# SysSec-KAIST/LTESniffer

Hardware: AMD Instinct MI355X
Metric: subframes/s (20 MHz, 150 RNTIs) (higher is better)
Workload: dtype f32+int16

## Files before the change

ltesniffer_amd/csrc/kernels/lsn_dsp.h:

```cpp
#pragma once
#include "lsn_dev.h"

__device__ __forceinline__ cf32 cmul(cf32 a, cf32 b) { cf32 c; c.r = a.r * b.r - a.i * b.i; c.i = a.r * b.i + a.i * b.r; return c; }
__device__ __forceinline__ cf32 cmulconj(cf32 a, cf32 b) { cf32 c; c.r = a.r * b.r + a.i * b.i; c.i = a.i * b.r - a.r * b.i; return c; }
__device__ __forceinline__ float cabs2(cf32 a) { return a.r * a.r + a.i * a.i; }

template <int R>
__device__ __forceinline__ void fft_pass(cf32* a, const cf32* w, int s, int N, int lgN, int tid)
{
  constexpr int G = 1 << R;
  const int h = 1 << s;
#pragma unroll
  for (int u = 0; u < (8 >> R); u++) {
    int g = tid * (8 >> R) + u;
    if (g >= (N >> R)) break;
    int low = g & (h - 1), high = g >> s, base = (high << (s + R)) | low;
    cf32 e[G];
#pragma unroll
    for (int j = 0; j < G; j++) e[j] = a[base + j * h];
#pragma unroll
    for (int q = 0; q < R; q++) {
#pragma unroll
      for (int j = 0; j < G; j++) {
        if (j & (1 << q)) continue;
        int pos = low + (j & ((1 << q) - 1)) * h;
        cf32 v = cmul(e[j + (1 << q)], w[pos << (lgN - (s + q + 1))]);
        cf32 uu = e[j];
        e[j].r = uu.r + v.r; e[j].i = uu.i + v.i;
        e[j + (1 << q)].r = uu.r - v.r; e[j + (1 << q)].i = uu.i - v.i;
      }
    }
#pragma unroll
    for (int j = 0; j < G; j++) a[base + j * h] = e[j];
  }
}
template <int NB>
__device__ __forceinline__ void fft_passes(cf32* a, const cf32* w, int M, int lgN, int tid)
{
  for (int s = 0; s < lgN;) {
    const int left = lgN - s;
    if (left >= 3) { for (int r = 0; r < NB; r++) fft_pass<3>(a + r * M, w, s, M, lgN, tid); s += 3; }
    else if (left == 2) { for (int r = 0; r < NB; r++) fft_pass<2>(a + r * M, w, s, M, lgN, tid); s += 2; }
    else { for (int r = 0; r < NB; r++) fft_pass<1>(a + r * M, w, s, M, lgN, tid); s += 1; }
    __syncthreads();
  }
}
template <typename Load>
__device__ __forceinline__ void lsn_symbol_fft(const LsnCellDev& c, cf32* a, cf32* w, Load load, cf32* out, int dc, int tid)
{
  const int N = (int)c.N, lgN = (int)c.lgN, nre = (int)c.nre;
  if (c.twiddle3) {
    const int M = (int)c.nsub;
    for (int n = tid; n < M / 2; n += 256) w[n] = c.twiddle[n];
    for (int n = tid; n < N; n += 256) {
      const cf32 x = load(n);
      const int m = n / 3, r = n - 3 * m;
      a[r * M + (int)(__brev((unsigned)m) >> (32 - lgN))] = x;
    }
    __syncthreads();
    fft_passes<3>(a, w, M, lgN, tid);
    const cf32* __restrict__ T = c.twiddle3;
    for (int k = tid; k < nre; k += 256) {
      const int bin = (k < nre / 2) ? (N - nre / 2 + k) : (k - nre / 2 + dc), kq = bin & (M - 1);
      int b2 = 2 * bin;
      b2 = b2 >= N ? b2 - N : b2;
      const cf32 t1 = cmul(a[M + kq], T[bin]), t2 = cmul(a[2 * M + kq], T[b2]);
      const float sr = a[kq].r + t1.r, si = a[kq].i + t1.i;
      cf32 X;
      X.r = sr + t2.r;
      X.i = si + t2.i;
      out[k] = X;
    }
    return;
  }
  for (int n = tid; n < N / 2; n += 256) w[n] = c.twiddle[n];
  for (int n = tid; n < N; n += 256) a[__brev((unsigned)n) >> (32 - lgN)] = load(n);
  __syncthreads();
  fft_passes<1>(a, w, N, lgN, tid);
  for (int k = tid; k < nre; k += 256) out[k] = a[(k < nre / 2) ? (N - nre / 2 + k) : (k - nre / 2 + dc)];
}

__device__ __forceinline__ void lsn_demod_llr(int Qm, float I, float Q, float* L)
{
  float aI = fabsf(I), aQ = fabsf(Q);
  L[0] = -I; L[1] = -Q;
  if (Qm == 4) {
    const float a = 0.31622776601683794f;
    L[2] = aI - 2.0f * a; L[3] = aQ - 2.0f * a;
  } else if (Qm == 6) {
    const float a = 0.15430334996209191f;
    float tI = aI - 4.0f * a, tQ = aQ - 4.0f * a;
    L[2] = tI; L[3] = tQ; L[4] = fabsf(tI) - 2.0f * a; L[5] = fabsf(tQ) - 2.0f * a;
  } else if (Qm == 8) {
    const float a = 0.07669649888473704f;
    float tI = aI - 8.0f * a, tQ = aQ - 8.0f * a;
    float uI = fabsf(tI) - 4.0f * a, uQ = fabsf(tQ) - 4.0f * a;
    L[2] = tI; L[3] = tQ; L[4] = uI; L[5] = uQ; L[6] = fabsf(uI) - 2.0f * a; L[7] = fabsf(uQ) - 2.0f * a;
  }
}
```

ltesniffer_amd/csrc/kernels/stage_a.hip:

```cpp
#include "lsn_dsp.h"
#include <algorithm>
#include <type_traits>
#include <cstdlib>

#define SQRT2F 1.41421356237309504880f

__device__ __forceinline__ void ofdm_rb_power(const LsnCellDev& c, const cf32* out, float* __restrict__ rbp_part, int sf, int l, int tid)
{
  __syncthreads();
  if (tid < (int)c.nof_prb) {
    float s = 0.0f;
    for (int k = 0; k < 12; k++) { const cf32 x = out[tid * 12 + k]; s = s + (x.r * x.r + x.i * x.i); }
    rbp_part[((size_t)sf * 14 + l) * 128 + tid] = s / 12.0f;
  }
}
__global__ __launch_bounds__(256) void k_ofdm(LsnCellDev c, const cf32* __restrict__ iq, const uint32_t* __restrict__ dphi_sf,
                                              cf32* __restrict__ grid, float* __restrict__ rbp_part)
{
  extern __shared__ __attribute__((aligned(16))) unsigned char smem[];
  const int N = (int)c.N, tid = threadIdx.x;
  cf32* a = (cf32*)smem;
  cf32* w = a + N;
  const int nsym = (int)c.nsym;
  const int blk = blockIdx.x, l = blk % nsym, rx = (blk / nsym) % (int)c.nof_rx, sf = blk / (nsym * (int)c.nof_rx);
  const int cp0 = 160 * N / 2048, cp1 = 144 * N / 2048;
  const int slot = l / 7, ls = l % 7;
  const int pos = c.cp ? l * (N + N / 4) + N / 4 : slot * (cp0 + 6 * cp1 + 7 * N) + cp0 + ls * (N + cp1);
  const cf32* in = iq + ((size_t)sf * c.iq_nant + rx) * c.sflen + pos;
  const uint32_t dphi = dphi_sf ? dphi_sf[sf] : 0u;
  const int nre = (int)c.nre;
  cf32* out = grid + (((size_t)sf * c.nof_rx + rx) * 14 + l) * nre;
  auto load = [&](int n) {
    cf32 x = in[n];
    if (dphi != 0u) {
      uint32_t ph = (uint32_t)(pos + n) * dphi;
      cf32 rot = cmul(c.nco_coarse[ph >> 20], c.nco_fine[(ph >> 10) & 1023u]);
      x = cmul(x, rot);
    }
    return x;
  };
  lsn_symbol_fft(c, a, w, load, out, 1, tid);
  if (rbp_part && rx == 0) ofdm_rb_power(c, out, rbp_part, sf, l, tid);
}

void lsn_launch_ofdm(const LsnCellDev& c, const cf32* iq, const uint32_t* dphi, cf32* grid, uint32_t nsf, hipStream_t s, float* rbp_part)
{
  size_t lds = sizeof(cf32) * (c.N + c.N / 2);
  LSN_LAUNCH(k_ofdm, dim3(nsf * c.nof_rx * c.nsym), dim3(256), lds, s, c, iq, dphi, grid, rbp_part);
}

__device__ __forceinline__ int crs_koff(const LsnCellDev& c, int port, int s)
{
  int v = (port == 0) ? ((s & 1) ? 3 : 0) : (port == 1) ? ((s & 1) ? 0 : 3) : (port == 2) ? 3 * s : 3 + 3 * s;
  return (v + (int)(c.id % 6)) % 6;
}

__global__ __launch_bounds__(256) void k_chest(LsnCellDev c, const cf32* __restrict__ grid, const uint32_t* __restrict__ sf_idx_arr,
                                               cf32* __restrict__ ce, float* __restrict__ raw)
{
  extern __shared__ __attribute__((aligned(16))) unsigned char smem[];
  const int nre = (int)c.nre, nref = (int)c.nref, tid = threadIdx.x;
  const int P = (int)c.nof_ports, A = (int)c.nof_rx;
  const int blk = blockIdx.x, p = blk % P, rx = (blk / P) % A, sf = blk / (P * A);
  cf32* ls = (cf32*)smem;
  cf32* sm = ls + 4 * nref;
  float* part = (float*)(sm + 4 * nref);
  const int S = p < 2 ? 4 : 2;
  const int nsl = (int)c.nslot, nsym = (int)c.nsym;
  const int sym[4] = {p < 2 ? 0 : 1, p < 2 ? nsl - 3 : nsl + 1, nsl, 2 * nsl - 3};
  const cf32* g = grid + ((size_t)sf * A + rx) * 14 * nre;
  const cf32* crs = c.crs + ((size_t)sf_idx_arr[sf] * P + p) * 4 * nref;
  const int n4 = S * nref;
  for (int i = tid; i < n4; i += 256) {
    int s = i / nref, m = i - s * nref;
    ls[i] = cmulconj(g[sym[s] * nre + 6 * m + crs_koff(c, p, s)], crs[i]);
  }
  __syncthreads();
  for (int i = tid; i < n4; i += 256) {
    int s = i / nref, m = i - s * nref;
    float ar = 0.0f, ai = 0.0f;
#pragma unroll
    for (int j = 0; j < 5; j++) {
      int q = m + j - 2;
      if (q < 0 || q >= nref) continue;
      ar = ar + c.taps[j] * ls[s * nref + q].r;
      ai = ai + c.taps[j] * ls[s * nref + q].i;
    }
    sm[i].r = ar; sm[i].i = ai;
  }
  __syncthreads();
  float p0 = 0.0f, p1 = 0.0f, p2 = 0.0f, p3 = 0.0f, p4 = 0.0f, p5 = 0.0f;
  for (int i = tid; i < n4; i += 256) {
    float dr = sm[i].r - ls[i].r, di = sm[i].i - ls[i].i;
    p0 = p0 + (dr * dr + di * di);
    p1 = p1 + ls[i].r;
    p2 = p2 + ls[i].i;
    p3 = p3 + (sm[i].r * sm[i].r + sm[i].i * sm[i].i);
  }
  if (p < 2)
    for (int i = tid; i < 2 * nref; i += 256) {
      cf32 t = (i < nref) ? cmulconj(ls[2 * nref + i], ls[i]) : cmulconj(ls[3 * nref + (i - nref)], ls[nref + (i - nref)]);
      p4 = p4 + t.r;
      p5 = p5 + t.i;
    }
  part[0 * 256 + tid] = p0; part[1 * 256 + tid] = p1; part[2 * 256 + tid] = p2;
  part[3 * 256 + tid] = p3; part[4 * 256 + tid] = p4; part[5 * 256 + tid] = p5;
  __syncthreads();
  for (int s = 128; s > 0; s >>= 1) {
    if (tid < s) {
#pragma unroll
      for (int q = 0; q < 6; q++) part[q * 256 + tid] = part[q * 256 + tid] + part[q * 256 + tid + s];
    }
    __syncthreads();
  }
  if (tid < 6) raw[(((size_t)sf * A + rx) * P + p) * 8 + tid] = part[tid * 256];
  cf32* co = ce + (((size_t)sf * P + p) * A + rx) * 14 * nre;
  for (int k = tid; k < nre; k += 256) {
    cf32 row[4];
#pragma unroll
    for (int s = 0; s < 4; s++) {
      if (s >= S) break;
      int koff = crs_koff(c, p, s);
      const cf32* pl = sm + s * nref;
      int m = (k - koff) >= 0 ? (k - koff) / 6 : 0;
      if (m > nref - 2) m = nref - 2;
      float dr = (pl[m + 1].r - pl[m].r) / 6.0f, di = (pl[m + 1].i - pl[m].i) / 6.0f;
      float f = (float)(k - (6 * m + koff));
      row[s].r = pl[m].r + dr * f;
      row[s].i = pl[m].i + di * f;
    }
    if (p >= 2) {
      const cf32 c1 = row[0], c8 = row[1];
      const int la = sym[0], lb = sym[1];
      const float dl = (float)(lb - la);
      const float dr = (c8.r - c1.r) / dl, di = (c8.i - c1.i) / dl;
      co[la * nre + k] = c1; co[lb * nre + k] = c8;
      for (int l = 0; l < nsym; l++) {
        if (l == la || l == lb) continue;
        cf32 v; v.r = c1.r + dr * (float)(l - la); v.i = c1.i + di * (float)(l - la); co[l * nre + k] = v;
      }
      continue;
    }
    cf32 c0 = row[0], c4 = row[1], c7 = row[2], c11 = row[3];
    const int q0 = sym[0], q1 = sym[1], q2 = sym[2], q3 = sym[3];
    const float w01 = (float)(q1 - q0), w12 = (float)(q2 - q1), w23 = (float)(q3 - q2);
    float d01r = (c4.r - c0.r) / w01, d01i = (c4.i - c0.i) / w01;
    float d12r = (c7.r - c4.r) / w12, d12i = (c7.i - c4.i) / w12;
    float d23r = (c11.r - c7.r) / w23, d23i = (c11.i - c7.i) / w23;
    co[q0 * nre + k] = c0; co[q1 * nre + k] = c4; co[q2 * nre + k] = c7; co[q3 * nre + k] = c11;
    for (int l = q0 + 1; l < q1; l++) { cf32 v; v.r = c0.r + d01r * (float)(l - q0); v.i = c0.i + d01i * (float)(l - q0); co[l * nre + k] = v; }
    for (int l = q1 + 1; l < q2; l++) { cf32 v; v.r = c4.r + d12r * (float)(l - q1); v.i = c4.i + d12i * (float)(l - q1); co[l * nre + k] = v; }
    for (int l = q2 + 1; l < q3; l++) { cf32 v; v.r = c7.r + d23r * (float)(l - q2); v.i = c7.i + d23i * (float)(l - q2); co[l * nre + k] = v; }
    for (int l = q3 + 1; l < nsym; l++) { cf32 v; v.r = c11.r + d23r * (float)(l - q3); v.i = c11.i + d23i * (float)(l - q3); co[l * nre + k] = v; }
  }
}

void lsn_launch_chest(const LsnCellDev& c, const cf32* grid, const uint32_t* sf_idx, cf32* ce, float* raw, uint32_t nsf, hipStream_t s)
{
  size_t lds = sizeof(cf32) * 8 * c.nref + sizeof(float) * 6 * 256;
  LSN_LAUNCH(k_chest, dim3(nsf * c.nof_rx * c.nof_ports), dim3(256), lds, s, c, grid, sf_idx, ce, raw);
}

__global__ void k_chest_fin(LsnCellDev c, const float* __restrict__ raw, LsnChest* __restrict__ out, uint32_t nsf)
{
  uint32_t sf = blockIdx.x * blockDim.x + threadIdx.x;
  if (sf >= nsf) return;
  const int A = (int)c.nof_rx, P = (int)c.nof_ports;
  LsnChest o;
  float ns = 0.0f, rs = 0.0f, cp = 0.0f, cr = 0.0f, ci = 0.0f;
  for (int q = 0; q < LSN_MAX_RX * LSN_MAX_PORTS; q++) { o.noise[q] = 0.0f; o.rsrp[q] = 0.0f; o.cepow[q] = 0.0f; }
  for (int rx = 0; rx < A; rx++)
    for (int p = 0; p < P; p++) {
      const float* r = raw + (((size_t)sf * A + rx) * P + p) * 8;
      const float n = (float)((p < 2 ? 4 : 2) * c.nref);
      float noise = r[0] / n, mr = r[1] / n, mi = r[2] / n, cepow = r[3] / n;
      float rsrp = mr * mr + mi * mi;
      o.noise[rx * P + p] = noise; o.rsrp[rx * P + p] = rsrp; o.cepow[rx * P + p] = cepow;
      ns = ns + noise; rs = rs + rsrp; cp = cp + cepow;
      cr = cr + r[4]; ci = ci + r[5];
    }
  float cnt = (float)(A * P);
  o.noise_avg = ns / cnt; o.rsrp_avg = rs / cnt; o.chan_ref = cp; o.corr_r = cr; o.corr_i = ci;
  o.pad[0] = o.pad[1] = o.pad[2] = 0.0f;
  out[sf] = o;
}
void lsn_launch_chest_fin(const LsnCellDev& c, const float* raw, LsnChest* out, uint32_t nsf, hipStream_t s)
{
  LSN_LAUNCH(k_chest_fin, dim3((nsf + 63) / 64), dim3(64), 0, s, c, raw, out, nsf);
}

__device__ __forceinline__ void reg_equalise(const LsnCellDev& c, const cf32* __restrict__ g, const cf32* __restrict__ ce, float noise,
                                             int l, int k0, cf32* x, int rs, int ps)
{
  const int A = (int)c.nof_rx;
  int kk[4], n = 0;
  if ((c.reg_w6 >> l) & 1u) {
    for (int k = k0; k < k0 + 6; k++)
      if ((k % 3) != (int)(c.id % 3)) { if (n < 4) kk[n] = k; n++; }
  } else {
    for (int k = 0; k < 4; k++) kk[k] = k0 + k;
  }
  if (c.nof_ports == 1) {
#pragma unroll
    for (int i = 0; i < 4; i++) {
      float nr = 0.0f, ni = 0.0f, den = 0.0f;
      for (int rx = 0; rx < A; rx++) {
        cf32 y = g[rx * rs + kk[i]];
        cf32 h = ce[rx * rs + kk[i]];
        cf32 t = cmulconj(y, h);
        float hp = h.r * h.r + h.i * h.i;
        if (rx == 0) { nr = t.r; ni = t.i; den = hp; } else { nr = nr + t.r; ni = ni + t.i; den = den + hp; }
      }
      den = den + noise;
      x[i].r = nr / den; x[i].i = ni / den;
    }
  } else {
#pragma unroll
    for (int i = 0; i < 4; i += 2) {
      float x0r = 0, x0i = 0, x1r = 0, x1i = 0, hh = 0;
      const int pa = (c.nof_ports == 4 && i == 2) ? 1 : 0, pb = c.nof_ports == 4 ? pa + 2 : 1;
      for (int rx = 0; rx < A; rx++) {
        const int bg = rx * rs, b0 = pa * ps + rx * rs, b1 = pb * ps + rx * rs;
        cf32 r0 = g[bg + kk[i]], r1 = g[bg + kk[i + 1]];
        cf32 h00 = ce[b0 + kk[i]], h01 = ce[b0 + kk[i + 1]], h10 = ce[b1 + kk[i]], h11 = ce[b1 + kk[i + 1]];
        float hp = (h00.r * h00.r + h00.i * h00.i) + (h11.r * h11.r + h11.i * h11.i);
        cf32 a = cmulconj(r0, h00), b = cmulconj(h11, r1), cc = cmulconj(h10, r0), d = cmulconj(r1, h01);
        float t0r = a.r + b.r, t0i = a.i + b.i, t1r = d.r - cc.r, t1i = d.i - cc.i;
        if (rx == 0) { x0r = t0r; x0i = t0i; x1r = t1r; x1i = t1i; hh = hp; }
        else { x0r = x0r + t0r; x0i = x0i + t0i; x1r = x1r + t1r; x1i = x1i + t1i; hh = hh + hp; }
      }
      x[i].r = x0r / hh * SQRT2F; x[i].i = x0i / hh * SQRT2F;
      x[i + 1].r = x1r / hh * SQRT2F; x[i + 1].i = x1i / hh * SQRT2F;
    }
  }
}

__global__ __launch_bounds__(64) void k_pcfich(LsnCellDev c, const cf32* __restrict__ grid, const cf32* __restrict__ ce,
                                               const LsnChest* __restrict__ ch, const uint32_t* __restrict__ sf_idx_arr,
                                               uint32_t* __restrict__ cfi_out, float* __restrict__ corr_out)
{
  __shared__ float llr[32];
  const int sf = blockIdx.x, lane = threadIdx.x;
  const cf32* g = grid + (size_t)sf * c.nof_rx * 14 * c.nre;
  const cf32* e = ce + (size_t)sf * c.nof_ports * c.nof_rx * 14 * c.nre;
  const uint8_t* scr = c.pcfich_scr + sf_idx_arr[sf] * 32;
  if (lane < 4) {
    cf32 x[4];
    reg_equalise(c, g, e, ch[sf].noise_avg, 0, (int)c.pcfich_k0[lane], x, 14 * (int)c.nre, (int)c.nof_rx * 14 * (int)c.nre);
    for (int j = 0; j < 4; j++) {
      float a = -(x[j].r * SQRT2F), b = -(x[j].i * SQRT2F);
      llr[8 * lane + 2 * j] = scr[8 * lane + 2 * j] ? -a : a;
      llr[8 * lane + 2 * j + 1] = scr[8 * lane + 2 * j + 1] ? -b : b;
    }
  }
  __syncthreads();
  if (lane == 0) {
    uint32_t best = 0; float bestc = 0.0f;
    for (int w = 0; w < 3; w++) {
      float acc = 0.0f;
      for (int i = 0; i < 32; i++) acc = acc + (((i % 3) != w) ? llr[i] : -llr[i]);
      corr_out[sf * 3 + w] = acc;
      if (w == 0 || acc > bestc) { bestc = acc; best = (uint32_t)w; }
    }
    cfi_out[sf] = best + 1;
  }
}
void lsn_launch_pcfich(const LsnCellDev& c, const cf32* grid, const cf32* ce, const LsnChest* ch, const uint32_t* sf_idx, uint32_t* cfi, float* corr, uint32_t nsf, hipStream_t s)
{
  LSN_LAUNCH(k_pcfich, dim3(nsf), dim3(64), 0, s, c, grid, ce, ch, sf_idx, cfi, corr);
}

__global__ __launch_bounds__(256) void k_pdcch_llr(LsnCellDev c, const cf32* __restrict__ grid, const cf32* __restrict__ ce,
                                                   const LsnChest* __restrict__ ch, const uint32_t* __restrict__ sf_idx_arr,
                                                   const uint32_t* __restrict__ cfi_arr, float* __restrict__ llr)
{
  const int sf = blockIdx.y;
  const uint32_t cfi = cfi_arr[sf];
  const int nre = (int)c.nre, A = (int)c.nof_rx, n0 = nre / 6, n1 = nre / 4;
  const int nat = blockIdx.x * 256 + threadIdx.x;
  int l = 0, k0 = 0, r = nat;
  for (;; l++) {
    const int six = (int)((c.reg_w6 >> l) & 1u), cnt = six ? n0 : n1;
    if (r < cnt || l == 3) { k0 = (six ? 6 : 4) * r; break; }
    r -= cnt;
  }
  if (k0 >= nre) return;
  if ((uint32_t)l >= cfi + (c.nof_prb <= 10 ? 1u : 0u) || nat >= 800) return;
  const uint32_t q = c.reg_q[(cfi - 1) * 800 + nat];
  if (q >= c.nof_cce[cfi - 1] * 9) return;
  const cf32* g = grid + ((size_t)sf * A * 14 + l) * nre;
  const cf32* e = ce + ((size_t)sf * c.nof_ports * A * 14 + l) * nre;
  const uint8_t* sc = c.pdcch_scr + (size_t)sf_idx_arr[sf] * LSN_LLR_STRIDE + 8 * q;
  cf32 x[4];
  reg_equalise(c, g, e, ch[sf].noise_avg, l, k0, x, 14 * nre, A * 14 * nre);
  float v[8];
#pragma unroll
  for (int j = 0; j < 4; j++) {
    float a = -(x[j].r * SQRT2F), b = -(x[j].i * SQRT2F);
    v[2 * j] = sc[2 * j] ? -a : a;
    v[2 * j + 1] = sc[2 * j + 1] ? -b : b;
  }
  float4 o0, o1;
  o0.x = v[0]; o0.y = v[1]; o0.z = v[2]; o0.w = v[3]; o1.x = v[4]; o1.y = v[5]; o1.z = v[6]; o1.w = v[7];
  float4* o = reinterpret_cast<float4*>(llr + (size_t)sf * LSN_LLR_STRIDE + 8 * q);
  o[0] = o0; o[1] = o1;
}
void lsn_launch_pdcch_llr(const LsnCellDev& c, const cf32* grid, const cf32* ce, const LsnChest* ch, const uint32_t* sf_idx, const uint32_t* cfi, float* llr, uint32_t nsf, hipStream_t s)
{
  const uint32_t nreg = c.nre / 6 + (c.nof_prb <= 10 ? 3u : 2u) * (c.nre / 4);
  LSN_LAUNCH(k_pdcch_llr, dim3((nreg + 255) / 256, nsf), dim3(256), 0, s, c, grid, ce, ch, sf_idx, cfi, llr);
}

__global__ __launch_bounds__(128) void k_cce_power(LsnCellDev c, const float* __restrict__ llr, const uint32_t* __restrict__ cfi_arr,
                                                   float* __restrict__ pw)
{
  const int sf = blockIdx.x, cce = threadIdx.x;
  if (cce >= LSN_CCE_STRIDE) return;
  float out = 0.0f;
  if ((uint32_t)cce < c.nof_cce[cfi_arr[sf] - 1]) {
    const float* l = llr + (size_t)sf * LSN_LLR_STRIDE + 72 * cce;
    double mean = 0.0;
    for (int i = 0; i < 72; i++) mean += (double)fabsf(l[i]);
    out = (float)(mean / 72.0);
  }
  pw[sf * LSN_CCE_STRIDE + cce] = out;
}
void lsn_launch_cce_power(const LsnCellDev& c, const float* llr, const uint32_t* cfi, float* pw, uint32_t nsf, hipStream_t s)
{
  LSN_LAUNCH(k_cce_power, dim3(nsf), dim3(128), 0, s, c, llr, cfi, pw);
}

__device__ __forceinline__ uint32_t ss_validate(uint32_t n, uint32_t ncce, uint32_t l, uint32_t nsubframe, uint32_t rnti)
{
  const bool ue = rnti >= 0x000Bu && rnti <= 0xFFF3u;
  if (!ue && !((rnti >= 1u && rnti <= 10u) || rnti >= 0xFFFDu)) return 0;
  uint32_t Yk = rnti;
  if (ue)
    for (uint32_t m = 0; m <= nsubframe; m++) {
      const uint32_t x = 39827u * Yk;
      const int t = (int)(x & 0xFFFFu) - (int)(x >> 16);
      Yk = (uint32_t)(t < 0 ? t + 65537 : t);
    }
  auto member = [&](uint32_t lv) -> bool {
    const uint32_t L = 1u << lv;
    if (n < L) return false;
    if (lv >= 2) {
      const uint32_t lim = (n < 16u ? n : 16u) / L;
      if ((ncce & (L - 1)) == 0 && ncce / L < lim && ncce + L <= n) return true;
    }
    if (!ue || (ncce & (L - 1))) return false;
// ... 499 lines not shown
```

ltesniffer_amd/csrc/kernels/stage_ul.hip:

```cpp
#include "lsn_dsp.h"

#define LLR_Q 180.0f

__global__ __launch_bounds__(256) void k_ul_fft(LsnCellDev c, const cf32* __restrict__ iq, uint32_t nant, uint32_t ant, cf32* __restrict__ grid)
{
  extern __shared__ __attribute__((aligned(16))) unsigned char smem[];
  const int N = (int)c.N, tid = threadIdx.x;
  cf32* a = (cf32*)smem;
  cf32* w = a + N;
  const int nsym = (int)c.nsym;
  const int l = blockIdx.x % nsym, sf = blockIdx.x / nsym;
  const int cp0 = 160 * N / 2048, cp1 = 144 * N / 2048;
  const int slot = l / 7, ls = l % 7;
  const int pos = c.cp ? l * (N + N / 4) + N / 4 : slot * (cp0 + 6 * cp1 + 7 * N) + cp0 + ls * (N + cp1);
  const cf32* in = iq + ((size_t)sf * nant + ant) * c.sflen + pos;
  const int nre = (int)c.nre;
  cf32* out = grid + ((size_t)sf * 14 + l) * nre;
  lsn_symbol_fft(c, a, w, [&](int n) { return cmul(in[n], c.ul_shift[n]); }, out, 0, tid);
}

void lsn_launch_ul_fft(const LsnCellDev& c, const cf32* iq, uint32_t nant, uint32_t ant, cf32* grid, uint32_t nsf, hipStream_t s)
{
  LSN_LAUNCH(k_ul_fft, dim3(nsf * c.nsym), dim3(256), sizeof(cf32) * (c.N + c.N / 2), s, c, iq, nant, ant, grid);
}

__global__ __launch_bounds__(256) void k_pusch_chest(LsnCellDev c, const LsnUlGrantDev* __restrict__ grants, const cf32* __restrict__ grid,
                                                     cf32* __restrict__ hs_out, float* __restrict__ stat)
{
  extern __shared__ __attribute__((aligned(16))) unsigned char smem[];
  const LsnUlGrantDev g = grants[blockIdx.x];
  const int M = 12 * (int)g.L_prb, nre = (int)c.nre, tid = threadIdx.x;
  cf32* ls = (cf32*)smem;
  float* part = (float*)(ls + 2 * M);
  for (int i = tid; i < 2 * M; i += 256) {
    const int s = i >= M ? 1 : 0, n = i - s * M;
    const cf32 y = grid[((size_t)g.sf * 14 + (c.nslot - 4) + c.nslot * s) * nre + 12 * (s ? g.n_prb2 : g.n_prb) + n];
    const cf32 r = cmul(c.ul_base[(s ? g.base_off1 : g.base_off) + n], c.ul_ph12[(g.ncs[s] * (uint32_t)n) % 12u]);
    ls[i] = cmulconj(y, r);
  }
  __syncthreads();
  cf32* hs = hs_out + g.hs_off;
  float p0 = 0.0f, p1 = 0.0f;
  for (int i = tid; i < 2 * M; i += 256) {
    const int s = i >= M ? 1 : 0, n = i - s * M;
    const cf32* q = ls + s * M;
    cf32 a;
    if (n == 0) { a.r = (q[0].r + q[1].r) / 2.0f; a.i = (q[0].i + q[1].i) / 2.0f; }
    else if (n == M - 1) { a.r = (q[n - 1].r + q[n].r) / 2.0f; a.i = (q[n - 1].i + q[n].i) / 2.0f; }
    else { a.r = ((q[n - 1].r + q[n].r) + q[n + 1].r) / 3.0f; a.i = ((q[n - 1].i + q[n].i) + q[n + 1].i) / 3.0f; }
    hs[i] = a;
    const float dr = a.r - q[n].r, di = a.i - q[n].i;
    p0 = p0 + (dr * dr + di * di);
    p1 = p1 + (a.r * a.r + a.i * a.i);
  }
  part[tid] = p0; part[256 + tid] = p1;
  __syncthreads();
  for (int s = 128; s > 0; s >>= 1) {
    if (tid < s) { part[tid] = part[tid] + part[tid + s]; part[256 + tid] = part[256 + tid] + part[256 + tid + s]; }
    __syncthreads();
  }
  if (tid == 0) {
    stat[2 * blockIdx.x] = part[0] / (float)(2 * M);
    stat[2 * blockIdx.x + 1] = part[256] / (float)(2 * M);
  }
}

void lsn_launch_pusch_chest(const LsnCellDev& c, const LsnUlGrantDev* g, const cf32* grid, cf32* hs, float* stat, uint32_t ngrants, hipStream_t s)
{
  LSN_LAUNCH(k_pusch_chest, dim3(ngrants), dim3(256), sizeof(cf32) * 2 * 1200 + sizeof(float) * 512, s, c, g, grid, hs, stat);
}

__global__ __launch_bounds__(256) void k_pusch_demod(LsnCellDev c, const LsnUlGrantDev* __restrict__ grants, const cf32* __restrict__ grid,
                                                     const cf32* __restrict__ hs_all, const float* __restrict__ stat, int16_t* __restrict__ llr)
{
  extern __shared__ __attribute__((aligned(16))) unsigned char smem[];
  const LsnUlGrantDev g = grants[blockIdx.y];
  const int nsl = (int)c.nslot, dm = nsl - 4, ncol = 2 * (nsl - 1);
  const int col = blockIdx.x, l = col < dm ? col : (col < nsl - 1 + dm ? col + 1 : col + 2);
  const int M = 12 * (int)g.L_prb, nre = (int)c.nre, Qm = (int)g.qm, tid = threadIdx.x;
  cf32* xa = (cf32*)smem;
  cf32* xb = xa + M;
  cf32* w = xb + M;
  const cf32* y = grid + ((size_t)g.sf * 14 + l) * nre + 12 * (l >= nsl ? g.n_prb2 : g.n_prb);
  const cf32* h = hs_all + g.hs_off + (l >= nsl ? 1 : 0) * M;
  const cf32* wt = c.ul_idft + g.idft_off;
  const float noise = stat[2 * blockIdx.y];
  for (int n = tid; n < M; n += 256) {
    const cf32 hh = h[n], t = cmulconj(y[n], hh);
    const float den = (hh.r * hh.r + hh.i * hh.i) + noise;
    cf32 v; v.r = t.r / den; v.i = t.i / den;
    xa[n] = v;
    w[n] = wt[n];
  }
  __syncthreads();
  cf32 *in = xa, *out = xb;
  for (int n = M, s = 1; n > 1;) {
    const int r = (n % 4 == 0) ? 4 : (n % 2 == 0) ? 2 : (n % 3 == 0) ? 3 : 5;
    const int m = n / r, wr = M / r;
    for (int o = tid; o < M; o += 256) {
      const int q = o % s, rest = o / s, t = rest % r, p = rest / r;
      cf32 acc = cmul(in[q + s * p], w[0]);
      int wi = 0;
      for (int i = 1; i < r; i++) {
        wi += t * wr; wi = wi >= M ? wi - M : wi;
        const cf32 term = cmul(in[q + s * (p + m * i)], w[wi]);
        acc.r = acc.r + term.r; acc.i = acc.i + term.i;
      }
      out[o] = cmul(acc, w[(int)(((unsigned)p * (unsigned)t * (unsigned)s) % (unsigned)M)]);
    }
    __syncthreads();
    cf32* sw = in; in = out; out = sw;
    n = m; s *= r;
  }
  const float scale = g.scale;
  int16_t* e = llr + g.llr_off;
  for (int r = tid; r < M; r += 256) {
    const float ar = in[r].r, ai = in[r].i;
    int dcell; bool is_ack = false;
    {
      const int qri = (int)g.q_ri, qack = (int)g.q_ack, qcqi = (int)g.q_cqi;
      auto in_col = [&](int q, int slot) { const int i0 = (4 - slot) & 3; return q > i0 ? (q - 1 - i0) / 4 + 1 : 0; };
      int before = 0; bool is_ri = false;
#pragma unroll
      for (int slot = 0; slot < 4; slot++) {
        const int cc = c.cp ? (slot == 0 ? 0 : (slot == 1 ? 3 : (slot == 2 ? 5 : 8))) : (slot == 0 ? 1 : (slot == 1 ? 4 : (slot == 2 ? 7 : 10))), n = in_col(qri, slot), top = M - n;
        before += r > top ? r - top : 0;
        if (n && r >= top && cc < col) before += 1;
        if (n && r >= top && cc == col) is_ri = true;
        const int ca = c.cp ? (slot == 0 ? 1 : (slot == 1 ? 2 : (slot == 2 ? 6 : 7))) : (slot == 0 ? 2 : (slot == 1 ? 3 : (slot == 2 ? 8 : 9)));
        if (ca == col && r >= M - in_col(qack, slot) && in_col(qack, slot)) is_ack = true;
      }
      const int rank = r * ncol + col - before;
      dcell = (is_ri || rank < qcqi) ? -1 : rank - qcqi;
    }
    float Lb[8];
    lsn_demod_llr(Qm, ar * scale, ai * scale, Lb);
#pragma unroll
    for (int b = 0; b < 8; b++) {
      if (b >= Qm) break;
      float v = rintf(Lb[b] * LLR_Q);
      v = v > (float)LSN_LLR_CLIP ? (float)LSN_LLR_CLIP : v;
      v = v < (float)-LSN_LLR_CLIP ? (float)-LSN_LLR_CLIP : v;
      int q = (int)v;
      const uint32_t sidx = ((uint32_t)col * (uint32_t)M + (uint32_t)r) * (uint32_t)Qm + (uint32_t)b;
      const uint32_t cbit = (uint32_t)c.gold_x1[sidx] ^ (uint32_t)(__popc(c.gold_x2mask[sidx] & g.cinit) & 1);
      if (dcell >= 0) e[(uint32_t)dcell * (uint32_t)Qm + (uint32_t)b] = is_ack ? (int16_t)0 : (int16_t)(cbit ? -q : q);
    }
  }
}

void lsn_launch_pusch_demod(const LsnCellDev& c, const LsnUlGrantDev* g, const cf32* grid, const cf32* hs, const float* stat, int16_t* llr,
                            uint32_t ngrants, hipStream_t s)
{
  LSN_LAUNCH(k_pusch_demod, dim3(2 * (c.nslot - 1), ngrants), dim3(256), sizeof(cf32) * 3 * 1200, s, c, g, grid, hs, stat, llr);
}

#define LSN_NZC 839

__device__ __forceinline__ void tree256_2(float* pr, float* pi, int tid)
{
  __syncthreads();
  for (int s = 128; s > 0; s >>= 1) {
    if (tid < s) { pr[tid] = pr[tid] + pr[tid + s]; pi[tid] = pi[tid] + pi[tid + s]; }
    __syncthreads();
  }
}

__global__ __launch_bounds__(256) void k_prach_bins(const cf32* __restrict__ iq, const uint64_t* __restrict__ occ_off, const cf32* __restrict__ W,
                                                    int N12, int Ncp, int b0, cf32* __restrict__ Y)
{
  __shared__ float pr[256], pi[256];
  const int j = blockIdx.x, o = blockIdx.y, tid = threadIdx.x;
  const cf32* x = iq + occ_off[o] + Ncp;
  const int b = ((b0 + j) % N12 + N12) % N12;
  int idx = (int)((long long)b * tid % N12);
  const int step = (int)((long long)b * 256 % N12);
  float ar = 0.0f, ai = 0.0f;
  for (int n = tid; n < N12; n += 256) {
    const cf32 p = cmul(x[n], W[idx]);
    ar = ar + p.r; ai = ai + p.i;
    idx += step; idx = idx >= N12 ? idx - N12 : idx;
  }
  pr[tid] = ar; pi[tid] = ai;
  tree256_2(pr, pi, tid);
  if (tid == 0) { cf32 y; y.r = pr[0]; y.i = pi[0]; Y[(size_t)o * LSN_NZC + j] = y; }
}

__global__ __launch_bounds__(256) void k_prach_corr(const cf32* __restrict__ Y, const cf32* __restrict__ D, const cf32* __restrict__ V, int nroots,
                                                    float* __restrict__ corr)
{
  __shared__ float pr[256], pi[256];
  const int k = blockIdx.x, root = blockIdx.y, o = blockIdx.z, tid = threadIdx.x;
  const cf32* y = Y + (size_t)o * LSN_NZC;
  const cf32* d = D + (size_t)root * LSN_NZC;
  float ar = 0.0f, ai = 0.0f;
  for (int j = tid; j < LSN_NZC; j += 256) {
    const cf32 p = cmul(cmulconj(y[j], d[j]), V[(j * k) % LSN_NZC]);
    ar = ar + p.r; ai = ai + p.i;
  }
  pr[tid] = ar; pi[tid] = ai;
  tree256_2(pr, pi, tid);
  if (tid == 0) corr[((size_t)o * nroots + root) * LSN_NZC + k] = pr[0] * pr[0] + pi[0] * pi[0];
}

__global__ __launch_bounds__(256) void k_prach_peaks(const float* __restrict__ corr, int nroots, int ncs, int nwin, float* __restrict__ out)
{
  __shared__ float pr[256], pi[256];
  const int root = blockIdx.x, o = blockIdx.y, tid = threadIdx.x;
  const float* c = corr + ((size_t)o * nroots + root) * LSN_NZC;
  float* res = out + ((size_t)o * nroots + root) * 130;
  float p = 0.0f;
  for (int i = tid; i < LSN_NZC; i += 256) p = p + c[i];
  pr[tid] = p; pi[tid] = 0.0f;
  tree256_2(pr, pi, tid);
  if (tid == 0) { res[0] = pr[0] / (float)LSN_NZC; res[1] = 0.0f; }
  if (tid < nwin && tid < 64) {
    const int start = (LSN_NZC - tid * ncs) % LSN_NZC, win = ncs ? ncs : LSN_NZC;
    float peak = 0.0f; int off = 0;
    for (int k = 0; k < win; k++) {
      const float v = c[start + k];
      if (v > peak) { peak = v; off = k; }
    }
    res[2 + 2 * tid] = peak; res[3 + 2 * tid] = (float)off;
  }
}

void lsn_launch_prach(const cf32* iq, const uint64_t* occ_off, uint32_t nocc, const cf32* W, const cf32* D, const cf32* V, int N12, int Ncp, int b0,
                      int nroots, int ncs, int nwin, cf32* Y, float* corr, float* out, hipStream_t s)
{
  if (!nocc) return;
  LSN_LAUNCH(k_prach_bins, dim3(LSN_NZC, nocc), dim3(256), 0, s, iq, occ_off, W, N12, Ncp, b0, Y);
  LSN_LAUNCH(k_prach_corr, dim3(LSN_NZC, nroots, nocc), dim3(256), 0, s, Y, D, V, nroots, corr);
  LSN_LAUNCH(k_prach_peaks, dim3(nroots, nocc), dim3(256), 0, s, corr, nroots, ncs, nwin, out);
}
```

Measured before the change: 284,800.

## Restructure OFDM FFT into compile-time pass plan with swizzled LDS and fused output

Replaces the runtime-looped radix FFT with templates specialised on log size, offering separate paths for power-of-two and 3x sizes. The first radix-8 stage now runs in registers straight from global loads, and a fixed sequence of passes follows. An XOR swizzle on LDS addresses is meant to avoid bank conflicts. Twiddles are read directly from global memory instead of being staged in shared memory, which cuts LDS size and barriers. The final pass writes subcarriers straight to the output and fills a per-RE power buffer for the RB power reduction, so the strided grid reread goes away. The trade-offs are more template instantiations and higher register pressure in the last pass.

```diff
diff --git a/ltesniffer_amd/csrc/kernels/lsn_dsp.h b/ltesniffer_amd/csrc/kernels/lsn_dsp.h
--- a/ltesniffer_amd/csrc/kernels/lsn_dsp.h
+++ b/ltesniffer_amd/csrc/kernels/lsn_dsp.h
@@ -1,83 +1,169 @@
 #pragma once
 #include "lsn_dev.h"
+#include "lsn_fft_map.h"
 
 __device__ __forceinline__ cf32 cmul(cf32 a, cf32 b) { cf32 c; c.r = a.r * b.r - a.i * b.i; c.i = a.r * b.i + a.i * b.r; return c; }
 __device__ __forceinline__ cf32 cmulconj(cf32 a, cf32 b) { cf32 c; c.r = a.r * b.r + a.i * b.i; c.i = a.i * b.r - a.r * b.i; return c; }
 __device__ __forceinline__ float cabs2(cf32 a) { return a.r * a.r + a.i * a.i; }
 
+template <int R, int S, int LG>
+__device__ __forceinline__ void fft_twiddles(cf32* tw, const cf32* __restrict__ W, int low)
+{
+#pragma unroll
+  for (int q = 0; q < R; q++)
+#pragma unroll
+    for (int m = 0; m < (1 << q); m++) tw[(1 << q) - 1 + m] = W[lsn_fft_twiddle(low + (m << S), S + q, LG)];
+}
 template <int R>
-__device__ __forceinline__ void fft_pass(cf32* a, const cf32* w, int s, int N, int lgN, int tid)
+__device__ __forceinline__ void fft_butterflies(cf32* e, const cf32* tw)
 {
-  constexpr int G = 1 << R;
-  const int h = 1 << s;
 #pragma unroll
-  for (int u = 0; u < (8 >> R); u++) {
-    int g = tid * (8 >> R) + u;
-    if (g >= (N >> R)) break;
-    int low = g & (h - 1), high = g >> s, base = (high << (s + R)) | low;
-    cf32 e[G];
+  for (int q = 0; q < R; q++) {
 #pragma unroll
-    for (int j = 0; j < G; j++) e[j] = a[base + j * h];
+    for (int j = 0; j < (1 << R); j++) {
+      if (j & (1 << q)) continue;
+      cf32 v = cmul(e[j + (1 << q)], tw[(1 << q) - 1 + (j & ((1 << q) - 1))]);
+      cf32 uu = e[j];
+      e[j].r = uu.r + v.r; e[j].i = uu.i + v.i;
+      e[j + (1 << q)].r = uu.r - v.r; e[j + (1 << q)].i = uu.i - v.i;
+    }
+  }
+}
+template <int R, int S, int LG, int NB>
+__device__ __forceinline__ void fft_pass(cf32* a, const cf32* __restrict__ W, int tid)
+{
+  constexpr int G = 1 << R, NG = NB << (LG - R);
 #pragma unroll
-    for (int q = 0; q < R; q++) {
+  for (int u = 0; u < (NG + LSN_FFT_THREADS - 1) / LSN_FFT_THREADS; u++) {
+    const int gg = tid + LSN_FFT_THREADS * u;
+    if (gg < NG) {
+      const int r = NB == 1 ? 0 : gg >> (LG - R), g = gg & ((1 << (LG - R)) - 1), base = lsn_fft_base(g, S, R);
+      const int at = lsn_fft_store(r, base, LG);
+      cf32 e[G], tw[G - 1];
+#pragma unroll
+      for (int j = 0; j < G; j++) e[j] = a[at ^ lsn_fft_slot(j << S)];
+      fft_twiddles<R, S, LG>(tw, W, base & ((1 << S) - 1));
+      fft_butterflies<R>(e, tw);
+#pragma unroll
+      for (int j = 0; j < G; j++) a[at ^ lsn_fft_slot(j << S)] = e[j];
+    }
+  }
+}
+template <int R, int LG>
+__device__ __forceinline__ void fft_last_pass(cf32* a, const cf32* __restrict__ W, cf32* __restrict__ out, float* pw, int nre, int dc, int tid)
+{
+  constexpr int G = 1 << R, S = LG - R, NG = 1 << S, U = (NG + LSN_FFT_THREADS - 1) / LSN_FFT_THREADS;
+  cf32 e[U][G], tw[U][G - 1];
+#pragma unroll
+  for (int u = 0; u < U; u++) {
+    const int g = tid + LSN_FFT_THREADS * u;
+    if (g < NG) {
+      const int at = lsn_fft_store(0, g, LG);
+#pragma unroll
+      for (int j = 0; j < G; j++) e[u][j] = a[at ^ lsn_fft_slot(j << S)];
+      fft_twiddles<R, S, LG>(tw[u], W, g);
+    }
+  }
+  if (pw) __syncthreads();
+#pragma unroll
+  for (int u = 0; u < U; u++) {
+    const int g = tid + LSN_FFT_THREADS * u;
+    if (g < NG) {
+      fft_butterflies<R>(e[u], tw[u]);
 #pragma unroll
       for (int j = 0; j < G; j++) {
-        if (j & (1 << q)) continue;
-        int pos = low + (j & ((1 << q) - 1)) * h;
-        cf32 v = cmul(e[j + (1 << q)], w[pos << (lgN - (s + q + 1))]);
-        cf32 uu = e[j];
-        e[j].r = uu.r + v.r; e[j].i = uu.i + v.i;
-        e[j + (1 << q)].r = uu.r - v.r; e[j + (1 << q)].i = uu.i - v.i;
+        const int k = lsn_fft_carrier(g + (j << S), 1 << LG, nre, dc);
+        if (k >= 0) {
+          out[k] = e[u][j];
+          if (pw) pw[k] = e[u][j].r * e[u][j].r + e[u][j].i * e[u][j].i;
+        }
       }
     }
-#pragma unroll
-    for (int j = 0; j < G; j++) a[base + j * h] = e[j];
   }
 }
-template <int NB>
-__device__ __forceinline__ void fft_passes(cf32* a, const cf32* w, int M, int lgN, int tid)
+template <int LG, int NB, typename Load>
+__device__ __forceinline__ void fft_run(const LsnCellDev& c, cf32* a, Load load, cf32* __restrict__ out, float* pw, int dc, int tid)
 {
-  for (int s = 0; s < lgN;) {
-    const int left = lgN - s;
-    if (left >= 3) { for (int r = 0; r < NB; r++) fft_pass<3>(a + r * M, w, s, M, lgN, tid); s += 3; }
-    else if (left == 2) { for (int r = 0; r < NB; r++) fft_pass<2>(a + r * M, w, s, M, lgN, tid); s += 2; }
-    else { for (int r = 0; r < NB; r++) fft_pass<1>(a + r * M, w, s, M, lgN, tid); s += 1; }
+  constexpr int M = 1 << LG, N = NB * M;
+  const cf32* __restrict__ W = c.twiddle;
+  const int nre = (int)c.nre;
+  if (tid < N / 8) {
+    cf32 x[8], e[8], tw[7];
+#pragma unroll
+    for (int jj = 0; jj < 8; jj++) x[jj] = load(lsn_fft_first_sample(tid, jj, N));
+#pragma unroll
+    for (int j = 0; j < 8; j++) e[j] = x[lsn_fft_brev3(j)];
+    fft_twiddles<3, 0, LG>(tw, W, 0);
+    fft_butterflies<3>(e, tw);
+    int r, g;
+    lsn_fft_first_group(tid, NB, LG, &r, &g);
+    const int at = lsn_fft_store(r, 8 * g, LG);
+#pragma unroll
+    for (int j = 0; j < 8; j++) a[at ^ lsn_fft_slot(j)] = e[j];
+  }
+  __syncthreads();
+  constexpr int R1 = LG >= 6 ? 3 : LG - 3, S2 = 3 + R1, R2 = LG - S2 >= 3 ? 3 : LG - S2, S3 = S2 + R2, R3 = LG - S3;
+  static_assert(LG >= 7 && LG <= 11 && R2 >= 1 && R3 >= 0 && R3 <= 2, "pass plan");
+  static_assert(R1 == 3 && (R3 == 0 || R2 == 3), "pass plan");
+  fft_pass<R1, 3, LG, NB>(a, W, tid);
+  __syncthreads();
+  if constexpr (R3 > 0) {
+    fft_pass<R2, S2, LG, NB>(a, W, tid);
     __syncthreads();
+  }
+  constexpr int RL = R3 > 0 ? R3 : R2, SL = LG - RL;
+  if constexpr (NB == 1) {
+    fft_last_pass<RL, LG>(a, W, out, pw, nre, dc, tid);
+  } else {
+    fft_pass<RL, SL, LG, NB>(a, W, tid);
+    __syncthreads();
+    const cf32* __restrict__ T = c.twiddle3;
+    float p[6];
+#pragma unroll
+    for (int it = 0; it < 6; it++) {
+      const int k = tid + LSN_FFT_THREADS * it;
+      if (k < nre) {
+        const int bin = lsn_fft_carrier_bin(k, N, nre, dc), kq = bin & (M - 1);
+        int b2 = 2 * bin;
+        b2 = b2 >= N ? b2 - N : b2;
+        const cf32 f0 = a[lsn_fft_store(0, kq, LG)];
+        const cf32 t1 = cmul(a[lsn_fft_store(1, kq, LG)], T[bin]), t2 = cmul(a[lsn_fft_store(2, kq, LG)], T[b2]);
+        const float sr = f0.r + t1.r, si = f0.i + t1.i;
+        cf32 X;
+        X.r = sr + t2.r;
+        X.i = si + t2.i;
+        out[k] = X;
+        p[it] = X.r * X.r + X.i * X.i;
+      }
+    }
+    if (pw) {
+      __syncthreads();
+#pragma unroll
+      for (int it = 0; it < 6; it++) {
+        const int k = tid + LSN_FFT_THREADS * it;
+        if (k < nre) pw[k] = p[it];
+      }
+    }
   }
 }
 template <typename Load>
-__device__ __forceinline__ void lsn_symbol_fft(const LsnCellDev& c, cf32* a, cf32* w, Load load, cf32* out, int dc, int tid)
+__device__ __forceinline__ void lsn_symbol_fft(const LsnCellDev& c, cf32* a, Load load, cf32* out, float* pw, int dc, int tid)
 {
-  const int N = (int)c.N, lgN = (int)c.lgN, nre = (int)c.nre;
   if (c.twiddle3) {
-    const int M = (int)c.nsub;
-    for (int n = tid; n < M / 2; n += 256) w[n] = c.twiddle[n];
-    for (int n = tid; n < N; n += 256) {
-      const cf32 x = load(n);
-      const int m = n / 3, r = n - 3 * m;
-      a[r * M + (int)(__brev((unsigned)m) >> (32 - lgN))] = x;
-    }
-    __syncthreads();
-    fft_passes<3>(a, w, M, lgN, tid);
-    const cf32* __restrict__ T = c.twiddle3;
-    for (int k = tid; k < nre; k += 256) {
-      const int bin = (k < nre / 2) ? (N - nre / 2 + k) : (k - nre / 2 + dc), kq = bin & (M - 1);
-      int b2 = 2 * bin;
-      b2 = b2 >= N ? b2 - N : b2;
-      const cf32 t1 = cmul(a[M + kq], T[bin]), t2 = cmul(a[2 * M + kq], T[b2]);
-      const float sr = a[kq].r + t1.r, si = a[kq].i + t1.i;
-      cf32 X;
-      X.r = sr + t2.r;
-      X.i = si + t2.i;
-      out[k] = X;
+    switch ((int)c.lgN) {
+      case 7: fft_run<7, 3>(c, a, load, out, pw, dc, tid); break;
+      case 8: fft_run<8, 3>(c, a, load, out, pw, dc, tid); break;
+      default: fft_run<9, 3>(c, a, load, out, pw, dc, tid); break;
     }
     return;
   }
-  for (int n = tid; n < N / 2; n += 256) w[n] = c.twiddle[n];
-  for (int n = tid; n < N; n += 256) a[__brev((unsigned)n) >> (32 - lgN)] = load(n);
-  __syncthreads();
-  fft_passes<1>(a, w, N, lgN, tid);
-  for (int k = tid; k < nre; k += 256) out[k] = a[(k < nre / 2) ? (N - nre / 2 + k) : (k - nre / 2 + dc)];
+  switch ((int)c.lgN) {
+    case 7: fft_run<7, 1>(c, a, load, out, pw, dc, tid); break;
+    case 8: fft_run<8, 1>(c, a, load, out, pw, dc, tid); break;
+    case 9: fft_run<9, 1>(c, a, load, out, pw, dc, tid); break;
+    case 10: fft_run<10, 1>(c, a, load, out, pw, dc, tid); break;
+    default: fft_run<11, 1>(c, a, load, out, pw, dc, tid); break;
+  }
 }
 
 __device__ __forceinline__ void lsn_demod_llr(int Qm, float I, float Q, float* L)
diff --git a/ltesniffer_amd/csrc/kernels/lsn_fft_map.h b/ltesniffer_amd/csrc/kernels/lsn_fft_map.h
--- /dev/null
+++ b/ltesniffer_amd/csrc/kernels/lsn_fft_map.h
@@ -0,0 +1,53 @@
+#pragma once
+#include <stdint.h>
+#ifndef LSN_HD
+#ifdef __HIPCC__
+#define LSN_HD __host__ __device__ __forceinline__
+#else
+#define LSN_HD static inline
+#endif
+#endif
+
+#define LSN_FFT_THREADS 256
+
+LSN_HD int lsn_fft_radix(int lgM, int s) { return (s == 0 || lgM - s >= 3) ? 3 : lgM - s; }
+
+LSN_HD int lsn_fft_first_sample(int t, int jj, int N) { return t + (N >> 3) * jj; }
+LSN_HD int lsn_fft_brev3(int j) { return ((j & 1) << 2) | (j & 2) | ((j >> 2) & 1); }
+LSN_HD void lsn_fft_first_group(int t, int nb, int lgM, int* r, int* g)
+{
+  const int tt = nb == 3 ? t / 3 : t;
+  *r = nb == 3 ? t - 3 * tt : 0;
+#if defined(__has_builtin) && __has_builtin(__builtin_bitreverse32)
+  *g = (int)(__builtin_bitreverse32((uint32_t)tt) >> (35 - lgM));
+#else
+  int b = 0;
+  for (int k = 0; k < lgM - 3; k++) b |= ((tt >> k) & 1) << (lgM - 4 - k);
+  *g = b;
+#endif
+}
+
+LSN_HD int lsn_fft_groups(int nb, int lgM, int R) { return nb << (lgM - R); }
+LSN_HD int lsn_fft_base(int g, int s, int R) { return ((g >> s) << (s + R)) | (g & ((1 << s) - 1)); }
+LSN_HD int lsn_fft_twiddle(int pos, int stage, int lgM) { return pos << (lgM - stage - 1); }
+
+LSN_HD int lsn_fft_slot(int i) { return i ^ ((i >> 3) & 0x1C) ^ ((i >> 5) & 2) ^ ((i >> 7) & 0xF); }
+LSN_HD int lsn_fft_block_key(int r) { return (0x1A20 >> (5 * r)) & 31; }
+LSN_HD int lsn_fft_store(int r, int i, int lgM) { return (r << lgM) | (lsn_fft_slot(i) ^ lsn_fft_block_key(r)); }
+LSN_HD int lsn_fft_lds_slots(int N) { return N; }
+
+LSN_HD int lsn_fft_carrier(int bin, int N, int nre, int dc)
+{
+  const int hf = nre >> 1;
+  if (bin >= N - hf) return bin - (N - hf);
+  if (bin >= dc && bin < dc + hf) return bin - dc + hf;
+  return -1;
+}
+LSN_HD int lsn_fft_carrier_bin(int k, int N, int nre, int dc) { return k < (nre >> 1) ? N - (nre >> 1) + k : k - (nre >> 1) + dc; }
+LSN_HD void lsn_fft_last_owner(int bin, int lgM, int R, int* t, int* u, int* j)
+{
+  const int g = bin & ((1 << (lgM - R)) - 1);
+  *j = bin >> (lgM - R);
+  *t = g & (LSN_FFT_THREADS - 1);
+  *u = g >> 8;
+}
diff --git a/ltesniffer_amd/csrc/kernels/stage_a.hip b/ltesniffer_amd/csrc/kernels/stage_a.hip
--- a/ltesniffer_amd/csrc/kernels/stage_a.hip
+++ b/ltesniffer_amd/csrc/kernels/stage_a.hip
@@ -5,12 +5,15 @@
 
 #define SQRT2F 1.41421356237309504880f
 
-__device__ __forceinline__ void ofdm_rb_power(const LsnCellDev& c, const cf32* out, float* __restrict__ rbp_part, int sf, int l, int tid)
+__device__ __forceinline__ void ofdm_rb_power(const LsnCellDev& c, const float* pw, float* __restrict__ rbp_part, int sf, int l, int tid)
 {
   __syncthreads();
   if (tid < (int)c.nof_prb) {
+    const float4* q = (const float4*)(pw + tid * 12);
+    const float4 q0 = q[0], q1 = q[1], q2 = q[2];
+    const float v[12] = {q0.x, q0.y, q0.z, q0.w, q1.x, q1.y, q1.z, q1.w, q2.x, q2.y, q2.z, q2.w};
     float s = 0.0f;
-    for (int k = 0; k < 12; k++) { const cf32 x = out[tid * 12 + k]; s = s + (x.r * x.r + x.i * x.i); }
+    for (int k = 0; k < 12; k++) s = s + v[k];
     rbp_part[((size_t)sf * 14 + l) * 128 + tid] = s / 12.0f;
   }
 }
@@ -20,7 +23,6 @@
   extern __shared__ __attribute__((aligned(16))) unsigned char smem[];
   const int N = (int)c.N, tid = threadIdx.x;
   cf32* a = (cf32*)smem;
-  cf32* w = a + N;
   const int nsym = (int)c.nsym;
   const int blk = blockIdx.x, l = blk % nsym, rx = (blk / nsym) % (int)c.nof_rx, sf = blk / (nsym * (int)c.nof_rx);
   const int cp0 = 160 * N / 2048, cp1 = 144 * N / 2048;
@@ -39,13 +41,14 @@
     }
     return x;
   };
-  lsn_symbol_fft(c, a, w, load, out, 1, tid);
-  if (rbp_part && rx == 0) ofdm_rb_power(c, out, rbp_part, sf, l, tid);
+  float* pw = (rbp_part && rx == 0) ? (float*)smem : nullptr;
+  lsn_symbol_fft(c, a, load, out, pw, 1, tid);
+  if (pw) ofdm_rb_power(c, pw, rbp_part, sf, l, tid);
 }
 
 void lsn_launch_ofdm(const LsnCellDev& c, const cf32* iq, const uint32_t* dphi, cf32* grid, uint32_t nsf, hipStream_t s, float* rbp_part)
 {
-  size_t lds = sizeof(cf32) * (c.N + c.N / 2);
+  size_t lds = sizeof(cf32) * lsn_fft_lds_slots((int)c.N);
   LSN_LAUNCH(k_ofdm, dim3(nsf * c.nof_rx * c.nsym), dim3(256), lds, s, c, iq, dphi, grid, rbp_part);
 }
 
diff --git a/ltesniffer_amd/csrc/kernels/stage_ul.hip b/ltesniffer_amd/csrc/kernels/stage_ul.hip
--- a/ltesniffer_amd/csrc/kernels/stage_ul.hip
+++ b/ltesniffer_amd/csrc/kernels/stage_ul.hip
@@ -7,7 +7,6 @@
   extern __shared__ __attribute__((aligned(16))) unsigned char smem[];
   const int N = (int)c.N, tid = threadIdx.x;
   cf32* a = (cf32*)smem;
-  cf32* w = a + N;
   const int nsym = (int)c.nsym;
   const int l = blockIdx.x % nsym, sf = blockIdx.x / nsym;
   const int cp0 = 160 * N / 2048, cp1 = 144 * N / 2048;
@@ -16,12 +15,12 @@
   const cf32* in = iq + ((size_t)sf * nant + ant) * c.sflen + pos;
   const int nre = (int)c.nre;
   cf32* out = grid + ((size_t)sf * 14 + l) * nre;
-  lsn_symbol_fft(c, a, w, [&](int n) { return cmul(in[n], c.ul_shift[n]); }, out, 0, tid);
+  lsn_symbol_fft(c, a, [&](int n) { return cmul(in[n], c.ul_shift[n]); }, out, nullptr, 0, tid);
 }
 
 void lsn_launch_ul_fft(const LsnCellDev& c, const cf32* iq, uint32_t nant, uint32_t ant, cf32* grid, uint32_t nsf, hipStream_t s)
 {
-  LSN_LAUNCH(k_ul_fft, dim3(nsf * c.nsym), dim3(256), sizeof(cf32) * (c.N + c.N / 2), s, c, iq, nant, ant, grid);
+  LSN_LAUNCH(k_ul_fft, dim3(nsf * c.nsym), dim3(256), sizeof(cf32) * lsn_fft_lds_slots((int)c.N), s, c, iq, nant, ant, grid);
 }
 
 __global__ __launch_bounds__(256) void k_pusch_chest(LsnCellDev c, const LsnUlGrantDev* __restrict__ grants, const cf32* __restrict__ grid,
```

Result: faster. 290,500, median of 6 (+2.0%).
